# scrubbbbs/cbird

Hardware: AMD Instinct MI355X
Metric: Hamming comparisons/sec + images hashed/sec, 1M-image index, 1/2/4/8 MI355X (higher is better)
Workload: dtype u64 hashes as 64 x FP4 signs, f32 accumulate (find, exact) / u8+f32 (hash)

## Files before the change

### cbird_amd/csrc/hamm64_mfma.hip

```cpp
#include <algorithm>
#include <mutex>
#include <vector>

#include "cbh_internal.h"
#include "fp4_sign.h"

namespace cbh {
namespace {

typedef _Float16 h2 __attribute__((ext_vector_type(2)));

constexpr int kThreads = 256;
constexpr int kWaves = 4;
constexpr int kHT = 8;
constexpr int kG = 2;
constexpr float kC0 = 8388608.0f + 16448.0f + 2097152.0f;
constexpr int kScale15 = 0x8e8e8e8e;
constexpr uint32_t kQueue = 2048;
constexpr uint32_t kFlagMaskPre = (1u << 5) | (1u << 11) | (1u << 17) | (1u << 23);
constexpr int kScaleHalf = 0x7e7e7e7e;
constexpr int kScale5 = (int)0x84848484;
constexpr int kScale11 = (int)0x8a8a8a8a;
constexpr int kScale17 = (int)0x90909090;

__global__ __launch_bounds__(256) void k_expand_needles(const uint64_t* __restrict__ q, uint32_t nq,
                                                        uint32_t nq_pad, uint4* __restrict__ qx) {
  const uint32_t i = blockIdx.x * 256u + threadIdx.x;
  if (i >= 3u * nq_pad) return;
  const uint32_t* w = reinterpret_cast<const uint32_t*>(q);
  if (i < 2u * nq_pad) {
    qx[i] = fp4_expand32((i >> 1) < nq ? w[i] : 0u);
  } else {
    const uint32_t j = i - 2u * nq_pad;
    qx[i] = fp4_expand32(j < nq ? w[2u * j] ^ w[2u * j + 1u] : 0u);
  }
}

__device__ __forceinline__ h2 as_h2(float f) { return __builtin_bit_cast(h2, f); }
__device__ __forceinline__ uint32_t as_u32(float f) { return __builtin_bit_cast(uint32_t, f); }
__device__ __forceinline__ h2 pkmax3(h2 a, h2 b, h2 c) {
  return __builtin_elementwise_maximum(__builtin_elementwise_maximum(a, b), c);
}
__device__ __forceinline__ void wave_order() {
  asm volatile("" ::: "memory");
  __builtin_amdgcn_wave_barrier();
  asm volatile("" ::: "memory");
}

struct HitParams {
  uint32_t lo_key, hi_key, lo_zero, hi_zero, thresh, n, nq, keep0;
  const uint64_t* q;
  const uint32_t* ids;
  cbh_record* rec;
  unsigned long long cap;
  unsigned long long* total;
  const uint2* hay;
  const uint2* qmask;
};

constexpr uint32_t kOutCap = 128;
__device__ __forceinline__ void out_flush(uint32_t* s_out, uint32_t& nout, const HitParams& hp) {
  if (nout == 0) return;
  wave_order();
  const uint32_t lane = threadIdx.x & 63u;
  unsigned long long base = 0;
  if (lane == 0) base = atomicAdd(hp.total, (unsigned long long)nout);
  const uint32_t blo = (uint32_t)__builtin_amdgcn_readfirstlane((int)(uint32_t)base);
  const uint32_t bhi = (uint32_t)__builtin_amdgcn_readfirstlane((int)(uint32_t)(base >> 32));
  base = ((unsigned long long)bhi << 32) | blo;
  for (uint32_t k = lane; k < nout; k += 64u) {
    const uint2 r = *reinterpret_cast<const uint2*>(&s_out[2u * k]);
    if (base + k < hp.cap) hp.rec[base + k] = ((cbh_record)r.y << 32) | r.x;
  }
  wave_order();
  nout = 0;
}
__device__ __forceinline__ void out_push(uint32_t* s_out, uint32_t& nout, bool has, uint32_t qidx, uint32_t dist,
                                         uint32_t id, const HitParams& hp) {
  const uint64_t m = __builtin_amdgcn_ballot_w64(has);
  if (m == 0) return;
  const uint32_t c = (uint32_t)__popcll(m);
  if (nout + c > kOutCap) out_flush(s_out, nout, hp);
  if (has) {
    const uint32_t pos = nout + __builtin_amdgcn_mbcnt_hi((uint32_t)(m >> 32), __builtin_amdgcn_mbcnt_lo((uint32_t)m, 0u));
    *reinterpret_cast<uint2*>(&s_out[2u * pos]) = make_uint2(id, (qidx << 7) | dist);
  }
  nout += c;
}

__device__ __forceinline__ bool mask_ok(const HitParams& hp, uint32_t row, uint32_t qi, uint64_t nv) {
  if (!hp.qmask) return true;
  const uint2 hv = hp.hay[row], mk = hp.qmask[qi];
  return (((hv.x ^ (uint32_t)nv) & mk.x) | ((hv.y ^ (uint32_t)(nv >> 32)) & mk.y)) == 0;
}

__device__ __forceinline__ void handle_tile2(const v16f& c, uint32_t row0, uint32_t p, const HitParams& hp,
                                             uint32_t* s_queue, uint32_t* s_out, uint32_t& nout) {
  const uint32_t lane = threadIdx.x & 63u;
  {
    h2 m0 = {0, 0}, m1 = {0, 0};
#pragma unroll
    for (int g = 0; g < 16; g += 4) {
      m0 = pkmax3(m0, as_h2(c[g]), as_h2(c[g + 1]));
      m1 = pkmax3(m1, as_h2(c[g + 2]), as_h2(c[g + 3]));
    }
    const uint32_t tb = __builtin_bit_cast(uint32_t, __builtin_elementwise_maximum(m0, m1));
    if (__builtin_amdgcn_ballot_w64((tb << 16) >= hp.lo_key || tb >= hp.hi_key) == 0) return;
  }
  uint32_t cnt = 0;
#pragma unroll
  for (int g = 0; g < 16; ++g) {
    const uint32_t bits = as_u32(c[g]);
    const bool fh = bits >= hp.hi_key;
    const bool fl = (bits << 16) >= hp.lo_key;
    if (__builtin_amdgcn_ballot_w64(fh || fl) == 0) continue;
    const uint64_t mh = __builtin_amdgcn_ballot_w64(fh);
    if (fh)
      s_queue[cnt + __builtin_amdgcn_mbcnt_hi((uint32_t)(mh >> 32), __builtin_amdgcn_mbcnt_lo((uint32_t)mh, 0u))] =
          ((hp.hi_zero - (bits >> 16)) << 11) | (1u << 10) | ((uint32_t)g << 6) | lane;
    cnt += (uint32_t)__popcll(mh);
    const uint64_t ml = __builtin_amdgcn_ballot_w64(fl);
    if (fl)
      s_queue[cnt + __builtin_amdgcn_mbcnt_hi((uint32_t)(ml >> 32), __builtin_amdgcn_mbcnt_lo((uint32_t)ml, 0u))] =
          (((hp.lo_zero - (bits & 0xffffu)) >> 1) << 11) | ((uint32_t)g << 6) | lane;
    cnt += (uint32_t)__popcll(ml);
  }
  wave_order();
  for (uint32_t k0 = 0; k0 < cnt; k0 += 64u) {
    const uint32_t k = k0 + lane;
    const uint32_t e = s_queue[min(k, cnt - 1u)];
    const uint32_t src = e & 63u, g = (e >> 6) & 15u, field = (e >> 10) & 1u;
    const uint32_t rit = (g & 3u) + 8u * (g >> 2) + 4u * (src >> 5);
    const uint32_t row = row0 + rit;
    const uint32_t qi = p * 64u + field * 32u + (src & 31u);
    const uint32_t d = e >> 11;
    bool has = false;
    uint32_t id = 0;
    if (k < cnt && row < hp.n && qi < hp.nq) {
      const uint64_t nv = hp.q[qi];
      if (nv != 0 && d < hp.thresh && mask_ok(hp, row, qi, nv)) {
        id = hp.ids[row];
        has = id != 0 || hp.keep0;
      }
    }
    out_push(s_out, nout, has, qi, d, id, hp);
  }
  wave_order();
}

constexpr uint32_t kParkLanes = 16;
constexpr uint32_t kPark = kQueue - kParkLanes * 32u;
constexpr uint32_t kOutOff = kPark - 2u * kOutCap;
static_assert(kOutOff / 2u >= 63u + (kHT / kG) * 32u, "pending list: one-lane groups of a step");
static_assert(kOutOff / 2u >= 63u + kParkLanes * 32u, "pending list: a chunk of hit lanes");

template <int A, int B, int G>
__device__ __forceinline__ uint32_t or_regs(const v16f (&c)[G]) {
  static_assert(B - A >= 3, "range");
  uint32_t o = as_u32(c[A >> 4][A & 15]) | as_u32(c[(A + 1) >> 4][(A + 1) & 15]) | as_u32(c[(A + 2) >> 4][(A + 2) & 15]);
#pragma unroll
  for (int r = A + 3; r < B; r += 2)
    o |= as_u32(c[r >> 4][r & 15]) | (r + 1 < B ? as_u32(c[(r + 1) >> 4][(r + 1) & 15]) : 0u);
  return o;
}

template <bool PRE>
__global__ __launch_bounds__(kThreads, PRE ? 4 : 1) void k_hamm64_mfma(
    const uint2* __restrict__ hay, const uint32_t* __restrict__ ids, uint32_t n,
    const uint64_t* __restrict__ q, const uint4* __restrict__ qx, uint32_t nq, uint32_t n_pairs,
    uint32_t pairs_per_chunk, uint32_t thresh, cbh_record* __restrict__ rec,
    unsigned long long cap, unsigned long long* __restrict__ total, uint32_t keep0,
    const uint2* __restrict__ qmask, const uint4* __restrict__ qf) {
  constexpr int HT = kHT, G = kG;
  __shared__ uint32_t s_queue_[kWaves][kQueue];
  __shared__ uint2 s_hay_[PRE ? kWaves : 1][PRE ? HT * 32 : 1];
  __shared__ uint32_t s_out2_[PRE ? 1 : kWaves][PRE ? 1 : 2 * kOutCap];
  const uint32_t lane = threadIdx.x & 63u;
  const uint32_t wave = (uint32_t)__builtin_amdgcn_readfirstlane((int)(threadIdx.x >> 6));
  const uint32_t r = lane & 31u, half = lane >> 5;
  const uint32_t tile0 = (blockIdx.x * kWaves + wave) * HT;
  if (tile0 * 32u >= n) return;
  uint32_t* s_queue = s_queue_[wave];
  uint2* s_hay = s_hay_[PRE ? wave : 0];
  uint32_t* s_out = PRE ? s_queue + kOutOff : s_out2_[PRE ? 0 : wave];
  uint32_t nout = 0;

  v8i a[HT];
#pragma unroll
  for (int t = 0; t < HT; ++t) {
    const uint32_t row = (tile0 + t) * 32u + r;
    const uint2 hv = row < n ? hay[row] : make_uint2(0u, 0u);
    a[t] = fp4_operand(fp4_expand32(PRE ? hv.x ^ hv.y : (half ? hv.y : hv.x)));
    if (PRE && half == 0) s_hay[t * 32 + r] = hv;
  }
  wave_order();
  v16f c0;
#pragma unroll
  for (int g = 0; g < 16; ++g)
    c0[g] = PRE ? 8388608.0f + (float)((16u + (thresh - 1u)) * 266305u) : kC0;
  asm volatile("" : "+v"(c0));
  int scale_b = PRE ? (half ? kScale5 : kScaleHalf) : kScaleOne;
  int scale_b2 = PRE ? (half ? kScale17 : kScale11) : kScale15;
  asm volatile("" : "+v"(scale_b));
  asm volatile("" : "+v"(scale_b2));

  const uint32_t p0 = blockIdx.y * pairs_per_chunk;
  const uint32_t p1 = min(n_pairs, p0 + pairs_per_chunk);
  const uint4* __restrict__ qp = qx + ((size_t)p0 * 64u + r) * 2u + half;
  const uint32_t lo_zero = 0x4080u;
  const uint32_t hi_zero = 0x4B40u;
  const uint32_t lo_thr = lo_zero - 2u * (thresh - 1u);
  const uint32_t hi_thr = hi_zero - (thresh - 1u);
  const uint32_t lo_key = lo_thr << 16, hi_key = hi_thr << 16;
  const HitParams hp = {lo_key, hi_key, lo_zero, hi_zero, thresh, n, nq, keep0, q, ids, rec, cap, total, hay, qmask};

  uint32_t npend = 0;
  auto drain = [&](bool all) {
    wave_order();
    const uint32_t keep = all ? 0u : (npend & 63u);
    for (uint32_t k0 = keep; k0 < npend; k0 += 64u) {
      const uint32_t k = min(k0 + lane, npend - 1u);
      const uint32_t bits = s_queue[2u * k], w1 = s_queue[2u * k + 1u];
      const uint32_t g = w1 & 15u, tile = (w1 >> 4) & 7u, L = (w1 >> 7) & 63u, pp = p0 + 2u * (w1 >> 13);
      const uint32_t rit = (g & 3u) + 8u * (g >> 2) + 4u * (L >> 5);
      const uint32_t row = (tile0 + tile) * 32u + rit;
      uint32_t fields = ((bits >> 23) & 1u) ? 0xfu
                                            : (((bits >> 5) & 1u) | (((bits >> 11) & 1u) << 1) | (((bits >> 17) & 1u) << 2));
      if (row >= hp.n || k0 + lane >= npend) fields = 0;
      const uint2 hv = s_hay[tile * 32u + rit];
      while (__builtin_amdgcn_ballot_w64(fields != 0) != 0) {
        const uint32_t qi = pp * 64u + (uint32_t)__builtin_ctz(fields | 16u) * 32u + (L & 31u);
        bool has = false;
        uint32_t d = 0, id = 0;
        if (fields != 0 && qi < hp.nq) {
          const uint64_t nv = hp.q[qi];
          d = __popc(hv.x ^ (uint32_t)nv) + __popc(hv.y ^ (uint32_t)(nv >> 32));
          if (nv != 0 && d < hp.thresh && mask_ok(hp, row, qi, nv)) {
            id = hp.ids[row];
            has = id != 0 || hp.keep0;
          }
        }
        out_push(s_out, nout, has, qi, d, id, hp);
        fields &= fields - 1u;
      }
    }
    wave_order();
    npend = keep;
  };

  auto step = [&](const uint32_t p, const uint4& nA, const uint4& nB) __attribute__((always_inline)) {
    const v8i bA = fp4_operand(nA);
    const v8i bB = fp4_operand(nB);
#pragma unroll
    for (int t0 = 0; t0 < HT; t0 += G) {
      v16f c[G];
#pragma unroll
      for (int t = 0; t < G; ++t)
        c[t] = __builtin_amdgcn_mfma_scale_f32_32x32x64_f8f6f4(a[t0 + t], bA, c0, 4, 4, 0, kScaleOne,
                                                               0, scale_b);
#pragma unroll
      for (int t = 0; t < G; ++t)
        c[t] = __builtin_amdgcn_mfma_scale_f32_32x32x64_f8f6f4(a[t0 + t], bB, c[t], 4, 4, 0,
                                                               kScaleOne, 0, scale_b2);
      if constexpr (PRE) {
        constexpr int R = G * 16;
        constexpr int RA = R / 2 + 1;
        const uint32_t half0 = or_regs<0, RA, G>(c), half1 = or_regs<RA, R, G>(c);
        const uint32_t flags = (half0 | half1) & kFlagMaskPre;
        const uint64_t hm = __builtin_amdgcn_ballot_w64(flags != 0);
        if (hm != 0) {
          static_assert(R == 32, "the parking slots below are 32 registers");
          auto park4 = [&](uint32_t at, int t, int k) {
            *reinterpret_cast<float4*>(&s_queue[at + (uint32_t)(t * 16 + 4 * k)]) =
                make_float4(c[t][4 * k], c[t][4 * k + 1], c[t][4 * k + 2], c[t][4 * k + 3]);
          };
          auto park = [&](uint32_t at) {
#pragma unroll
            for (int t = 0; t < G; ++t)
#pragma unroll
              for (int k = 0; k < 4; ++k) park4(at, t, k);
          };
          const uint32_t w1c = ((uint32_t)t0 << 4) | (((p - p0) >> 1) << 13);
          auto list = [&](uint32_t at, uint32_t L, uint32_t ok) {
            uint32_t ln = lane;
            asm volatile("" : "+v"(ln));
            const uint32_t v = s_queue[at + ln];
            const bool pred = (v & kFlagMaskPre) != 0 && ((ok >> (ln & 31u)) & 1u) != 0u;
            const uint32_t bm = (uint32_t)(__builtin_amdgcn_ballot_w64(pred) & 0xffffffffull);
            if (pred && ln < (uint32_t)R) {
              *reinterpret_cast<uint2*>(&s_queue[2u * (npend + __builtin_amdgcn_mbcnt_lo(bm, 0u))]) =
                  make_uint2(v, ln | (w1c | (L << 7)));
            }
            npend += (uint32_t)__popc(bm);
          };
          if ((hm & (hm - 1)) == 0) {
            const uint64_t b0 = __builtin_amdgcn_ballot_w64((half0 & kFlagMaskPre) != 0);
            const uint64_t b1 = __builtin_amdgcn_ballot_w64((half1 & kFlagMaskPre) != 0);
            if (flags != 0) {
              if (b0) {
#pragma unroll
                for (int k = 0; k < 4; ++k) park4(kPark, 0, k);
              }
              park4(kPark, 1, 0);
              if (b1) {
#pragma unroll
                for (int k = 1; k < 4; ++k) park4(kPark, 1, k);
              }
            }
            const uint32_t ok = (b0 ? 0x000fffffu : 0u) | (b1 ? 0xffff0000u : 0u);
            wave_order();
            list(kPark, (uint32_t)__builtin_ctzll(hm), ok);
            wave_order();
          } else {
            uint64_t rest = hm;
            for (;;) {
              if (rest ? npend + kParkLanes * 32u > kOutOff / 2u : npend >= 64u) drain(false);
              if (!rest) break;
              uint64_t cm = rest;
              if ((uint32_t)__popcll(rest) > kParkLanes) {
                uint64_t rem = rest;
                for (uint32_t i = 0; i < kParkLanes; ++i) rem &= rem - 1;
                cm = rest ^ rem;
              }
              rest ^= cm;
              if ((cm >> lane) & 1ull)
                park(kPark + 32u * __builtin_amdgcn_mbcnt_hi((uint32_t)(cm >> 32), __builtin_amdgcn_mbcnt_lo((uint32_t)cm, 0u)));
              wave_order();
              uint32_t at = kPark;
              for (uint64_t m = cm; m; m &= m - 1, at += 32u) list(at, (uint32_t)__builtin_ctzll(m), 0xffffffffu);
              wave_order();
            }
          }
        }
      } else {
        h2 m0 = {0, 0}, m1 = {0, 0};
#pragma unroll
        for (int t = 0; t < G; ++t)
#pragma unroll
          for (int g = 0; g < 16; g += 4) {
            m0 = pkmax3(m0, as_h2(c[t][g]), as_h2(c[t][g + 1]));
            m1 = pkmax3(m1, as_h2(c[t][g + 2]), as_h2(c[t][g + 3]));
          }
        const uint32_t mb = __builtin_bit_cast(uint32_t, __builtin_elementwise_maximum(m0, m1));
        const bool hit = (mb << 16) >= lo_key || mb >= hi_key;
        if (__builtin_amdgcn_ballot_w64(hit) != 0) {
#pragma unroll
          for (int t = 0; t < G; ++t) handle_tile2(c[t], (tile0 + t0 + t) * 32u, p, hp, s_queue, s_out, nout);
        }
      }
    }
    if constexpr (PRE)
      if (npend >= 64u) drain(false);
  };

  if constexpr (PRE) {
    typedef unsigned v4u_t __attribute__((ext_vector_type(4)));
    const __amdgpu_buffer_rsrc_t rsrc = __builtin_amdgcn_make_buffer_rsrc(
        const_cast<uint4*>(qf + (size_t)p0 * 64u), 0, (int)0xffffffffu, 0x27000);
    const uint32_t voff = lane * 16u;
    auto ldt = [&](uint32_t rel, uint32_t partner) -> uint4 {
      const uint32_t pr = min(rel + partner, n_pairs - 1u - p0);
      const v4u_t v = __builtin_amdgcn_raw_buffer_load_b128(rsrc, (int)voff, (int)(pr * 1024u), 0);
      return make_uint4(v.x, v.y, v.z, v.w);
    };
    const uint32_t np = p1 - p0;
    uint4 a0 = ldt(0, 0), a1 = ldt(0, 1);
#pragma unroll 1
    for (uint32_t rel = 0; rel < np; rel += 4) {
      const uint4 b0 = ldt(min(rel + 2, np - 1), 0), b1 = ldt(min(rel + 2, np - 1), 1);
      step(p0 + rel, a0, a1);
      if (rel + 2 < np) {
        a0 = ldt(min(rel + 4, np - 1), 0);
        a1 = ldt(min(rel + 4, np - 1), 1);
        step(p0 + rel + 2, b0, b1);
      }
    }
    if (npend) drain(true);
  } else {
    uint4 x0 = qp[0], x1 = qp[64];
    uint32_t p = p0;
    for (; p + 1 < p1; p += 2) {
      const uint4 y0 = qp[128], y1 = qp[192];
      step(p, x0, x1);
      qp += 256;
      if (p + 2 < p1) {
        x0 = qp[0];
        x1 = qp[64];
      }
      step(p + 1, y0, y1);
    }
    if (p < p1) step(p, x0, x1);
  }
  out_flush(s_out, nout, hp);
}


constexpr uint32_t kFlagMask3 = (1u << 7) | (1u << 14) | (1u << 21);
constexpr int kScale7 = (int)0x86868686;
constexpr int kScale14 = (int)0x8d8d8d8d;

__device__ __forceinline__ void handle_tile3(const v16f& c, uint32_t row0, uint32_t p3, const HitParams& hp,
                                             uint32_t* s_queue, uint32_t* s_out, uint32_t& nout) {
  const uint32_t lane = threadIdx.x & 63u;
  uint32_t any = 0;
#pragma unroll
  for (int g = 0; g < 16; ++g) any |= as_u32(c[g]);
  if (__builtin_amdgcn_ballot_w64((any & kFlagMask3) != 0) == 0) return;
  const uint32_t b = hp.thresh - 1u;
#pragma unroll 1
  for (uint32_t f = 0; f < 3; ++f) {
    uint32_t cnt = 0;
#pragma unroll
    for (int g = 0; g < 16; ++g) {
      const uint32_t bits = as_u32(c[g]);
      const bool fl = (bits >> (7u + 7u * f)) & 1u;
      const uint64_t m = __builtin_amdgcn_ballot_w64(fl);
      if (m == 0) continue;
      if (fl)
        s_queue[cnt + __builtin_amdgcn_mbcnt_hi((uint32_t)(m >> 32), __builtin_amdgcn_mbcnt_lo((uint32_t)m, 0u))] =
            ((64u + b - ((bits >> (1u + 7u * f)) & 0x7fu)) << 12) | (f << 10) | ((uint32_t)g << 6) | lane;
      cnt += (uint32_t)__popcll(m);
    }
    wave_order();
    for (uint32_t k0 = 0; k0 < cnt; k0 += 64u) {
      const uint32_t k = k0 + lane;
      const uint32_t e = s_queue[min(k, cnt - 1u)];
      const uint32_t src = e & 63u, g = (e >> 6) & 15u, field = (e >> 10) & 3u, d = e >> 12;
      const uint32_t row = row0 + (g & 3u) + 8u * (g >> 2) + 4u * (src >> 5);
      const uint32_t qi = p3 * 96u + field * 32u + (src & 31u);
      const uint64_t nv = (k < cnt && row < hp.n && qi < hp.nq) ? hp.q[qi] : 0;
      bool has = false;
      uint32_t id = 0;
      if (nv != 0 && mask_ok(hp, row, qi, nv)) {
        id = hp.ids[row];
        has = id != 0 || hp.keep0;
      }
      out_push(s_out, nout, has, qi, d, id, hp);
    }
    wave_order();
  }
}

__global__ __launch_bounds__(kThreads, 2) void k_hamm64_mfma3(
    const uint2* __restrict__ hay, const uint32_t* __restrict__ ids, uint32_t n,
    const uint64_t* __restrict__ q, const uint4* __restrict__ qx, uint32_t nq, uint32_t n_triples,
    uint32_t triples_per_chunk, uint32_t thresh, cbh_record* __restrict__ rec,
    unsigned long long cap, unsigned long long* __restrict__ total, uint32_t keep0,
    const uint2* __restrict__ qmask) {
  constexpr int HT = kHT, G = kG;
  __shared__ uint32_t s_queue_[kWaves][16 * 64];
  __shared__ uint32_t s_out_[kWaves][2 * kOutCap];
  const uint32_t lane = threadIdx.x & 63u, wave = threadIdx.x >> 6;
  const uint32_t r = lane & 31u, half = lane >> 5;
  const uint32_t tile0 = (blockIdx.x * kWaves + wave) * HT;
  if (tile0 * 32u >= n) return;
  uint32_t* s_queue = s_queue_[wave];
  uint32_t* s_out = s_out_[wave];
  uint32_t nout = 0;

  v8i a[HT];
#pragma unroll
  for (int t = 0; t < HT; ++t) {
    const uint32_t row = (tile0 + t) * 32u + r;
    const uint2 hv = row < n ? hay[row] : make_uint2(0u, 0u);
    a[t] = fp4_operand(fp4_expand32(half ? hv.y : hv.x));
  }
  const uint32_t b = thresh - 1u;
  v16f c0;
#pragma unroll
  for (int g = 0; g < 16; ++g) c0[g] = 8388608.0f + (float)((64u + 2u * b) * 16513u);
  asm volatile("" : "+v"(c0));
  const HitParams hp = {0, 0, 0, 0, thresh, n, nq, keep0, q, ids, rec, cap, total, hay, qmask};

  const uint32_t p0 = blockIdx.y * triples_per_chunk;
  const uint32_t p1 = min(n_triples, p0 + triples_per_chunk);

  auto step = [&](const uint32_t p, const uint4& n0, const uint4& n1, const uint4& n2) __attribute__((always_inline)) {
    const v8i b0 = fp4_operand(n0), b1 = fp4_operand(n1), b2 = fp4_operand(n2);
#pragma unroll
    for (int t0 = 0; t0 < HT; t0 += G) {
      v16f c[G];
#pragma unroll
      for (int t = 0; t < G; ++t)
        c[t] = __builtin_amdgcn_mfma_scale_f32_32x32x64_f8f6f4(a[t0 + t], b0, c0, 4, 4, 0, kScaleOne, 0,
                                                               kScaleOne);
#pragma unroll
      for (int t = 0; t < G; ++t)
        c[t] = __builtin_amdgcn_mfma_scale_f32_32x32x64_f8f6f4(a[t0 + t], b1, c[t], 4, 4, 0, kScaleOne, 0,
                                                               kScale7);
#pragma unroll
      for (int t = 0; t < G; ++t)
        c[t] = __builtin_amdgcn_mfma_scale_f32_32x32x64_f8f6f4(a[t0 + t], b2, c[t], 4, 4, 0, kScaleOne, 0,
                                                               kScale14);
      if (__builtin_amdgcn_ballot_w64((or_regs<0, G * 16, G>(c) & kFlagMask3) != 0) != 0) {
#pragma unroll
        for (int t = 0; t < G; ++t) handle_tile3(c[t], (tile0 + t0 + t) * 32u, p, hp, s_queue, s_out, nout);
      }
    }
  };

  typedef unsigned v4u_t __attribute__((ext_vector_type(4)));
  const __amdgpu_buffer_rsrc_t rsrc = __builtin_amdgcn_make_buffer_rsrc(
      const_cast<uint4*>(qx + (size_t)p0 * 192u), 0, (int)0xffffffffu, 0x27000);
  const uint32_t voff = (2u * r + half) * 16u;
  auto ldt = [&](uint32_t rel, uint32_t tile) -> uint4 {
    const v4u_t v = __builtin_amdgcn_raw_buffer_load_b128(rsrc, (int)voff, (int)(rel * 3072u + tile * 1024u), 0);
    return make_uint4(v.x, v.y, v.z, v.w);
  };
  const uint32_t np = p1 - p0;
  uint4 x0 = ldt(0, 0), x1 = ldt(0, 1), x2 = ldt(0, 2);
#pragma unroll 1
  for (uint32_t rel = 0; rel < np; rel += 2) {
    const uint32_t ry = min(rel + 1, np - 1);
    const uint4 y0 = ldt(ry, 0), y1 = ldt(ry, 1), y2 = ldt(ry, 2);
    step(p0 + rel, x0, x1, x2);
    if (rel + 1 < np) {
      const uint32_t rx = min(rel + 2, np - 1);
      x0 = ldt(rx, 0);
      x1 = ldt(rx, 1);
      x2 = ldt(rx, 2);
      step(p0 + rel + 1, y0, y1, y2);
    }
  }
  out_flush(s_out, nout, hp);
}

constexpr uint32_t kProbeS = 2048;
constexpr int kProbeT = kProbeMaxThresh;

__device__ __forceinline__ uint32_t probe_mix(uint32_t x) {
  x = ((x >> 16) ^ x) * 0x45d9f3bu;
  x = ((x >> 16) ^ x) * 0x45d9f3bu;
  return (x >> 16) ^ x;
}
__global__ __launch_bounds__(256) void k_fold_probe(const uint2* __restrict__ hay, uint32_t n, const uint2* __restrict__ q,
                                                    uint32_t nq, uint32_t sh, uint32_t sq, uint32_t* __restrict__ counts) {
  __shared__ uint2 s_h[64];
  __shared__ uint32_t s_cnt[2 * kProbeT];
  const uint32_t t = threadIdx.x;
  if (t < 64) {
    const uint32_t i = blockIdx.y * 64u + t;
    s_h[t] = i < sh ? hay[sh == n ? i : probe_mix(i) % n] : make_uint2(0u, 0u);
  }
  if (t < 2 * kProbeT) s_cnt[t] = 0;
  __syncthreads();
  const uint32_t j = blockIdx.x * 256u + t;
  const uint32_t nslots = min(64u, sh - blockIdx.y * 64u);
  uint32_t cnt[kProbeT] = {}, cnt64[kProbeT] = {};
  if (j < sq) {
    const uint2 nv = q[sq == nq ? j : probe_mix(j ^ 0x9e3779b9u) % nq];
    const uint32_t f = nv.x ^ nv.y;
    for (uint32_t k = 0; k < nslots; ++k) {
      const uint2 hv = s_h[k];
      const uint32_t d = (uint32_t)__popc(f ^ hv.x ^ hv.y);
#pragma unroll
      for (int th = 0; th < kProbeT; ++th) cnt[th] += d < (uint32_t)(th + 1) ? 1u : 0u;
      if (d < (uint32_t)kProbeT) {
        const uint32_t d64 = (uint32_t)__popc(nv.x ^ hv.x) + (uint32_t)__popc(nv.y ^ hv.y);
#pragma unroll
        for (int th = 0; th < kProbeT; ++th) cnt64[th] += d64 < (uint32_t)(th + 1) ? 1u : 0u;
      }
    }
  }
#pragma unroll
  for (int th = 0; th < 2 * kProbeT; ++th) {
    uint32_t v = th < kProbeT ? cnt[th % kProbeT] : cnt64[th % kProbeT];
#pragma unroll
    for (int o = 32; o > 0; o >>= 1) v += __shfl_down(v, o);
    if ((t & 63u) == 0 && v) atomicAdd(&s_cnt[th], v);
  }
  __syncthreads();
  if (t < 2 * kProbeT && s_cnt[t]) atomicAdd(&counts[t], s_cnt[t]);
}

std::mutex g_probe_mu;
std::vector<uint32_t*> g_probe_free;
uint32_t* probe_slot_get() {
  {
    std::lock_guard<std::mutex> lk(g_probe_mu);
    if (!g_probe_free.empty()) {
      uint32_t* p = g_probe_free.back();
      g_probe_free.pop_back();
      return p;
    }
  }
  uint32_t* p = nullptr;
  if (hipHostMalloc(&p, 2 * kProbeT * sizeof(uint32_t)) != hipSuccess) {
    (void)hipGetLastError();
    return nullptr;
  }
  return p;
}
void probe_slot_put(uint32_t* p) {
  std::lock_guard<std::mutex> lk(g_probe_mu);
  g_probe_free.push_back(p);
}

}

bool probe_fold_rates(const uint64_t* d_hashes, size_t n, const uint64_t* d_q, size_t nq, int thresh, hipStream_t stream,
                      double* r_cand, double* r_true) {
  uint32_t* d_cnt = nullptr;
  if (cbh::malloc_async((void**)&d_cnt, 2 * kProbeT * sizeof(uint32_t), stream) != hipSuccess) {
    (void)hipGetLastError();
    return false;
  }
  uint32_t* h_cnt = probe_slot_get();
  bool ok = h_cnt != nullptr;
  const uint32_t sh = (uint32_t)std::min<size_t>(n, kProbeS), sq = (uint32_t)std::min<size_t>(nq, kProbeS);
  if (ok) {
    ok = hipMemsetAsync(d_cnt, 0, 2 * kProbeT * sizeof(uint32_t), stream) == hipSuccess;
    if (ok) {
      hipLaunchKernelGGL(k_fold_probe, dim3((sq + 255u) / 256u, (sh + 63u) / 64u), dim3(256), 0, stream,
                         reinterpret_cast<const uint2*>(d_hashes), (uint32_t)n, reinterpret_cast<const uint2*>(d_q),
                         (uint32_t)nq, sh, sq, d_cnt);
      ok = hipGetLastError() == hipSuccess &&
           hipMemcpyAsync(h_cnt, d_cnt, 2 * kProbeT * sizeof(uint32_t), hipMemcpyDeviceToHost, stream) == hipSuccess &&
           hipStreamSynchronize(stream) == hipSuccess;
    }
  }
  (void)cbh::free_async(d_cnt, stream);
  if (ok) {
    const double pairs = (double)sh * (double)sq;
    *r_cand = (double)h_cnt[thresh - 1] / pairs;
    *r_true = (double)h_cnt[kProbeT + thresh - 1] / pairs;
  } else {
    (void)hipGetLastError();
  }
  if (h_cnt) probe_slot_put(h_cnt);
  return ok;
}

static uint32_t padded_needles(size_t nq) { return (uint32_t)((nq + 191) / 192) * 192u; }

int expand_needles_for_scan(const uint64_t* d_q, size_t nq, hipStream_t stream, uint4** qx_out) {
  *qx_out = nullptr;
  if (nq == 0 || nq > CBH_MAX_QUERIES_PER_CALL) return CBH_OK;
  const uint32_t nq_pad = padded_needles(nq);
  uint4* qx = nullptr;
  CBH_HIP(malloc_async((void**)&qx, (size_t)nq_pad * 48u, stream));
  hipLaunchKernelGGL(k_expand_needles, dim3((3u * nq_pad + 255u) / 256u), dim3(256), 0, stream, d_q,
                     (uint32_t)nq, nq_pad, qx);
  hipError_t e = hipGetLastError();
  if (e != hipSuccess) {
    (void)free_async(qx, stream);
    CBH_HIP(e);
  }
  *qx_out = qx;
  return CBH_OK;
}

int launch_hamm64_scan_mfma(const uint64_t* d_hashes, const uint32_t* d_ids, size_t n, const uint64_t* d_q, size_t nq,
                            int thresh, cbh_record* d_rec, size_t cap, unsigned long long* d_total, hipStream_t stream,
                            bool pre, const ScanOpts& o) {
  const uint32_t n_pairs = (uint32_t)((nq + 63) / 64);
  const uint32_t n_triples = (uint32_t)((nq + 95) / 96);
  const uint32_t nq_pad = padded_needles(nq);
  const uint4* qx = o.qx;
  uint4* qx_own = nullptr;
  if (!qx) {
    int rc = expand_needles_for_scan(d_q, nq, stream, &qx_own);
    if (rc) return rc;
    qx = qx_own;
  }
  const uint4* qf = qx + 2u * (size_t)nq_pad;
  const uint32_t rows_per_wg = 32u * kHT * kWaves;
  const uint32_t sib = std::max(1u, o.siblings);
  const uint32_t wgs = (uint32_t)((n + rows_per_wg - 1) / rows_per_wg);
  if (!pre && thresh <= 64) {
    uint32_t tpc = 172u;
    while (tpc > 11 && (uint64_t)wgs * sib * ((n_triples + tpc - 1) / tpc) < 8192) tpc = (tpc + 1) / 2;
    uint32_t ch3 = (n_triples + tpc - 1) / tpc;
    if (ch3 > 65535) {
      tpc = (n_triples + 65534) / 65535;
      ch3 = (n_triples + tpc - 1) / tpc;
    }
    hipLaunchKernelGGL(k_hamm64_mfma3, dim3(wgs, ch3), dim3(kThreads), 0, stream,
                       reinterpret_cast<const uint2*>(d_hashes), d_ids, (uint32_t)n, d_q, qx, (uint32_t)nq, n_triples, tpc,
                       (uint32_t)thresh, d_rec, (unsigned long long)cap, d_total, (uint32_t)o.keep_id0,
                       reinterpret_cast<const uint2*>(o.d_qmask));
  } else {
    uint32_t ppc = pre ? 512u : 256u;
    while (ppc > 16 && (uint64_t)wgs * sib * ((n_pairs + ppc - 1) / ppc) < 8192) ppc >>= 1;
    uint32_t chunks = (n_pairs + ppc - 1) / ppc;
    if (chunks > 65535) {
      ppc = ((n_pairs + 65534) / 65535 + 1u) & ~1u;
      chunks = (n_pairs + ppc - 1) / ppc;
    }
#define CBH_MFMA(PRE)                                                                                                 \
  hipLaunchKernelGGL((k_hamm64_mfma<PRE>), dim3(wgs, chunks), dim3(kThreads), 0, stream,                              \
                     reinterpret_cast<const uint2*>(d_hashes), d_ids, (uint32_t)n, d_q, qx, (uint32_t)nq, n_pairs, ppc, \
                     (uint32_t)thresh, d_rec, (unsigned long long)cap, d_total, (uint32_t)o.keep_id0,                 \
                     reinterpret_cast<const uint2*>(o.d_qmask), qf)
    if (pre) CBH_MFMA(true); else CBH_MFMA(false);
#undef CBH_MFMA
  }
  hipError_t e = hipGetLastError();
  if (qx_own) (void)cbh::free_async(qx_own, stream);
  CBH_HIP(e);
  return CBH_OK;
}

}
```

### cbird_amd/csrc/hamm64_scan.hip

```cpp
#include <atomic>

#include "cbh_internal.h"

namespace cbh {
namespace {

constexpr int kThreads = 256;
constexpr int kH = 8;
constexpr int kQB = 8;

__device__ __forceinline__ uint32_t min3u(uint32_t a, uint32_t b, uint32_t c) {
  return min(min(a, b), c);
}

__device__ __forceinline__ void emit(cbh_record* __restrict__ rec, unsigned long long cap,
                                     unsigned long long* __restrict__ total, uint32_t qidx,
                                     uint32_t dist, uint32_t id) {
  unsigned long long slot = atomicAdd(total, 1ull);
  if (slot < cap) rec[slot] = ((cbh_record)qidx << 39) | ((cbh_record)dist << 32) | id;
}

template <int H>
__device__ __forceinline__ void exact_block(const uint2 (&h)[H], uint32_t base_idx, uint32_t n,
                                            const uint32_t* __restrict__ ids,
                                            const uint64_t* __restrict__ q, uint32_t qa,
                                            uint32_t qb, uint32_t thresh,
                                            cbh_record* __restrict__ rec, unsigned long long cap,
                                            unsigned long long* __restrict__ total,
                                            uint32_t keep0, const uint2* __restrict__ qmask) {
#pragma unroll 1
  for (uint32_t qi = qa; qi < qb; ++qi) {
    const uint64_t qq = q[qi];
    if (qq == 0) continue;
    const uint32_t ql = (uint32_t)qq, qh = (uint32_t)(qq >> 32);
    const uint2 mk = qmask ? qmask[qi] : make_uint2(0u, 0u);
#pragma unroll
    for (int j = 0; j < H; ++j) {
      const uint32_t d = __popc(h[j].x ^ ql) + __popc(h[j].y ^ qh);
      if (d < thresh && (((h[j].x ^ ql) & mk.x) | ((h[j].y ^ qh) & mk.y)) == 0) {
        const uint32_t idx = base_idx + (uint32_t)j * kThreads;
        if (idx < n) {
          const uint32_t id = ids[idx];
          if (id != 0 || keep0) emit(rec, cap, total, qi, d, id);
        }
      }
    }
  }
}

template <int H, int QB>
__device__ __forceinline__ void refine_block(const uint2 (&h)[H], const uint32_t (&acc)[H],
                                             const uint2 (&cur)[QB], uint32_t base_idx, uint32_t n,
                                             const uint32_t* __restrict__ ids, uint32_t qb,
                                             uint32_t thresh, cbh_record* __restrict__ rec,
                                             unsigned long long cap,
                                             unsigned long long* __restrict__ total,
                                             uint32_t keep0, const uint2* __restrict__ qmask) {
#pragma unroll
  for (int j = 0; j < H; ++j) {
    if (acc[j] < thresh) {
      const uint32_t idx = base_idx + (uint32_t)j * kThreads;
      uint32_t d[QB];
#pragma unroll
      for (int i = 0; i < QB; ++i) d[i] = __popc(h[j].x ^ cur[i].x) + __popc(h[j].y ^ cur[i].y);
      uint32_t m = d[0];
#pragma unroll
      for (int i = 1; i + 1 < QB; i += 2) m = min3u(m, d[i], d[i + 1]);
      if (QB % 2 == 0) m = min(m, d[QB - 1]);
      if (m < thresh && idx < n) {
        const uint32_t id = ids[idx];
        if (id != 0 || keep0) {
#pragma unroll
          for (int i = 0; i < QB; ++i)
            if (d[i] < thresh && (cur[i].x | cur[i].y) != 0) {
              const uint2 mk = qmask ? qmask[qb + (uint32_t)i] : make_uint2(0u, 0u);
              if ((((h[j].x ^ cur[i].x) & mk.x) | ((h[j].y ^ cur[i].y) & mk.y)) == 0)
                emit(rec, cap, total, qb + (uint32_t)i, d[i], id);
            }
        }
      }
    }
  }
}

enum { MODE_PRE = 0, MODE_FULL = 1, MODE_EQ = 2 };

template <int H, int QB, int MODE>
__global__ __launch_bounds__(kThreads) void k_hamm64_scan(
    const uint2* __restrict__ hay, const uint32_t* __restrict__ ids, uint32_t n,
    const uint64_t* __restrict__ q, uint32_t nq, uint32_t q_chunk, uint32_t thresh,
    cbh_record* __restrict__ rec, unsigned long long cap, unsigned long long* __restrict__ total,
    uint32_t keep0, const uint2* __restrict__ qmask) {
  const uint32_t base_idx = blockIdx.x * (uint32_t)(kThreads * H) + threadIdx.x;
  uint2 h[H];
#pragma unroll
  for (int j = 0; j < H; ++j) {
    const uint32_t idx = base_idx + (uint32_t)j * kThreads;
    h[j] = idx < n ? hay[idx] : make_uint2(0u, 0u);
  }
  const uint32_t q0 = blockIdx.y * q_chunk;
  const uint32_t q1 = min(nq, q0 + q_chunk);
  uint32_t qb = q0;
  const uint2* __restrict__ qp = reinterpret_cast<const uint2*>(q) + (size_t)q0;

  uint2 cur[QB];
  if (qb + QB <= q1) {
#pragma unroll
    for (int i = 0; i < QB; ++i) cur[i] = qp[i];
  }
  for (; qb + QB <= q1; qb += QB) {
    uint2 nxt[QB];
    qp += QB;
    if (qb + 2 * QB <= q1) {
#pragma unroll
      for (int i = 0; i < QB; ++i) nxt[i] = qp[i];
    } else {
#pragma unroll
      for (int i = 0; i < QB; ++i) nxt[i] = make_uint2(0u, 0u);
    }
    if (MODE == MODE_EQ) {
      unsigned long long any = 0;
#pragma unroll
      for (int i = 0; i < QB; ++i) {
        const unsigned long long qq = ((unsigned long long)cur[i].y << 32) | cur[i].x;
#pragma unroll
        for (int j = 0; j < H; ++j) {
          const unsigned long long hh = ((unsigned long long)h[j].y << 32) | h[j].x;
          any |= __ballot(hh == qq);
        }
      }
      if (any) exact_block<H>(h, base_idx, n, ids, q, qb, qb + QB, thresh, rec, cap, total, keep0, qmask);
    } else {
      uint32_t acc[H];
#pragma unroll
      for (int j = 0; j < H; ++j) acc[j] = 0xffu;
      uint32_t ql[QB], qh[QB];
#pragma unroll
      for (int i = 0; i < QB; ++i) {
        asm volatile("v_mov_b32 %0, %1" : "=v"(ql[i]) : "s"(cur[i].x));
        if (MODE == MODE_FULL) asm volatile("v_mov_b32 %0, %1" : "=v"(qh[i]) : "s"(cur[i].y));
      }
      uint32_t x[QB][H];
      __builtin_amdgcn_sched_barrier(0);
#pragma unroll
      for (int i = 0; i < QB; ++i)
#pragma unroll
        for (int j = 0; j < H; ++j) x[i][j] = h[j].x ^ ql[i];
      __builtin_amdgcn_sched_barrier(0);
      if (MODE == MODE_FULL) {
#pragma unroll
        for (int i = 0; i < QB; ++i)
#pragma unroll
          for (int j = 0; j < H; ++j) x[i][j] = (uint32_t)__popc(x[i][j]);
        uint32_t y[QB][H];
        __builtin_amdgcn_sched_barrier(0);
#pragma unroll
        for (int i = 0; i < QB; ++i)
#pragma unroll
          for (int j = 0; j < H; ++j) y[i][j] = h[j].y ^ qh[i];
        __builtin_amdgcn_sched_barrier(0);
#pragma unroll
        for (int i = 0; i < QB; i += 2)
#pragma unroll
          for (int j = 0; j < H; ++j)
            acc[j] = min3u(acc[j], x[i][j] + (uint32_t)__popc(y[i][j]),
                           x[i + 1][j] + (uint32_t)__popc(y[i + 1][j]));
      } else {
#pragma unroll
        for (int i = 0; i < QB; i += 2)
#pragma unroll
          for (int j = 0; j < H; ++j)
            acc[j] = min3u(acc[j], (uint32_t)__popc(x[i][j]), (uint32_t)__popc(x[i + 1][j]));
      }
      __builtin_amdgcn_sched_barrier(0);
      uint32_t m = acc[0];
#pragma unroll
      for (int j = 1; j + 1 < H; j += 2) m = min3u(m, acc[j], acc[j + 1]);
      if (H % 2 == 0) m = min(m, acc[H - 1]);
      if (m < thresh) refine_block<H, QB>(h, acc, cur, base_idx, n, ids, qb, thresh, rec, cap, total, keep0, qmask);
    }
#pragma unroll
    for (int i = 0; i < QB; ++i) cur[i] = nxt[i];
  }
  if (qb < q1) exact_block<H>(h, base_idx, n, ids, q, qb, q1, thresh, rec, cap, total, keep0, qmask);
}

constexpr unsigned kLoneSlots = 8;
__global__ __launch_bounds__(256) void k_find_one(const uint2* __restrict__ hay, const uint32_t* __restrict__ ids,
                                                  uint32_t n, uint32_t qlo, uint32_t qhi, uint32_t thresh,
                                                  unsigned* __restrict__ d_state, LoneBlock* __restrict__ host,
                                                  unsigned long long seq) {
  const uint32_t base = blockIdx.x * (256u * kLoneSlots) + threadIdx.x;
  bool wrote = false;
#pragma unroll
  for (unsigned k = 0; k < kLoneSlots; ++k) {
    const uint32_t i = base + k * 256u;
    if (i >= n) break;
    const uint2 hv = hay[i];
    const uint32_t d = (uint32_t)__popc(hv.x ^ qlo) + (uint32_t)__popc(hv.y ^ qhi);
    if (d < thresh) {
      const uint32_t id = ids[i];
      if (id != 0) {
        const unsigned slot = atomicAdd(&d_state[0], 1u);
        if (slot < LoneBlock::kRecs) {
          host->recs[slot] = ((cbh_record)d << 32) | id;
          wrote = true;
        }
      }
    }
  }
  if (wrote) __threadfence_system();
  __syncthreads();
  if (threadIdx.x == 0) {
    __threadfence();
    if (atomicAdd(&d_state[1], 1u) == gridDim.x - 1u) {
      __threadfence();
      host->count = atomicExch(&d_state[0], 0u);
      d_state[1] = 0u;
      __threadfence_system();
      __hip_atomic_store(const_cast<unsigned long long*>(&host->done), seq, __ATOMIC_RELEASE, __HIP_MEMORY_SCOPE_SYSTEM);
    }
  }
}

}

int launch_find_one(const uint64_t* d_hashes, const uint32_t* d_ids, size_t n, uint64_t q, int thresh, unsigned* d_state,
                    LoneBlock* h_block, unsigned long long seq, hipStream_t stream) {
  if (n == 0 || n > 0xfffffff0ull || !d_state || !h_block || thresh <= 0) return CBH_E_INVAL;
  const unsigned per_wg = 256u * kLoneSlots;
  hipLaunchKernelGGL(k_find_one, dim3((unsigned)((n + per_wg - 1) / per_wg)), dim3(256), 0, stream,
                     reinterpret_cast<const uint2*>(d_hashes), d_ids, (uint32_t)n, (uint32_t)q, (uint32_t)(q >> 32),
                     (uint32_t)thresh, d_state, h_block, seq);
  CBH_HIP(hipGetLastError());
  return CBH_OK;
}

int wait_find_one(const LoneBlock* h_block, unsigned long long seq, hipStream_t stream) {
  const unsigned long long* flag = const_cast<const unsigned long long*>(&h_block->done);
  for (unsigned spins = 0;; ++spins) {
    if (__atomic_load_n(flag, __ATOMIC_ACQUIRE) == seq) return CBH_OK;
    if ((spins & 0xfffu) == 0xfffu) {
      const hipError_t q = hipStreamQuery(stream);
      if (q == hipSuccess) {
        return __atomic_load_n(flag, __ATOMIC_ACQUIRE) == seq ? CBH_OK : CBH_E_HIP;
      }
      if (q != hipErrorNotReady) {
        set_last_error("k_find_one", q);
        return CBH_E_HIP;
      }
    }
#if defined(__x86_64__)
    __builtin_ia32_pause();
#endif
  }
}

namespace {

constexpr int kPreMax = 7;
constexpr size_t kMfmaMinNq = 256;
constexpr size_t kMfmaMinN = 4096;
constexpr int kPreStatic = 6;
constexpr double kTrueWeight = 4.0;
constexpr uint64_t kProbeMinPairs = 1ull << 31;

int g_scan_mfma = 1;
int g_pre_max_thresh = -1;
int g_pre_rate_max_e9 = 125000;
std::atomic<uint64_t> g_pre_mask{0};
std::atomic<uint64_t> g_n_probe{0};
std::atomic<long long> g_last_rate_e9{-1};
std::atomic<long long> g_last_true_e9{-1};

enum class Join { None, IfCheaper, Forced };
enum class Kernel { PopcEq, PopcPre, PopcFull, Mfma };
struct Route {
  Join join;
  Kernel kernel;
  double scan_ms;
};

Route route(size_t n, size_t nq, int thresh, bool masked) {
  Route r;
  r.scan_ms = (double)n * (double)nq * (thresh <= 6 ? 8.8e-12 : 16.3e-12);
  const bool joinable = thresh <= kJoinMaxThresh && !masked && n < 0xfffffff0ull;
  r.join = !joinable ? Join::None : g_scan_mfma == 4 ? Join::Forced
           : g_scan_mfma == 3 && r.scan_ms >= 1.0 ? Join::IfCheaper : Join::None;
  const bool mfma = thresh <= 65 && (g_scan_mfma == 2 || g_scan_mfma == 4 ||
                                     (g_scan_mfma != 0 && nq >= kMfmaMinNq && n >= kMfmaMinN));
  r.kernel = mfma ? Kernel::Mfma : thresh == 1 ? Kernel::PopcEq : thresh <= kPreMax ? Kernel::PopcPre : Kernel::PopcFull;
  return r;
}

int launch_popc(Kernel kernel, const uint64_t* d_hashes, const uint32_t* d_ids, size_t n, const uint64_t* d_q, size_t nq,
                int thresh, cbh_record* d_rec, size_t cap, unsigned long long* d_total, hipStream_t stream,
                const ScanOpts& o) {
  const uint32_t tile = kThreads * kH;
  const uint32_t tiles = (uint32_t)((n + tile - 1) / tile);
  uint32_t q_chunk = 16384;
  while (q_chunk > 1024 && (uint64_t)tiles * ((nq + q_chunk - 1) / q_chunk) < 8192) q_chunk >>= 1;
  uint32_t chunks = (uint32_t)((nq + q_chunk - 1) / q_chunk);
  if (chunks > 65535) {
    q_chunk = (uint32_t)((nq + 65534) / 65535);
    q_chunk = (q_chunk + kQB - 1) / kQB * kQB;
    chunks = (uint32_t)((nq + q_chunk - 1) / q_chunk);
  }
  dim3 grid(tiles, chunks), block(kThreads);
  const uint2* hay = reinterpret_cast<const uint2*>(d_hashes);
#define CBH_SCAN(MODE)                                                                                                  \
  hipLaunchKernelGGL((k_hamm64_scan<kH, kQB, MODE>), grid, block, 0, stream, hay, d_ids, (uint32_t)n, d_q, (uint32_t)nq, \
                     q_chunk, (uint32_t)thresh, d_rec, (unsigned long long)cap, d_total, (uint32_t)o.keep_id0,            \
                     reinterpret_cast<const uint2*>(o.d_qmask))
  if (kernel == Kernel::PopcEq) CBH_SCAN(MODE_EQ);
  else if (kernel == Kernel::PopcPre) CBH_SCAN(MODE_PRE);
  else CBH_SCAN(MODE_FULL);
#undef CBH_SCAN
  CBH_HIP(hipGetLastError());
  return CBH_OK;
}

}

bool scan_takes_mfma(size_t n, size_t nq, int thresh) {
  return thresh >= 1 && route(n, nq, thresh, false).kernel == Kernel::Mfma;
}

bool scan_pick_pre(const uint64_t* d_hashes, size_t n, size_t n_total, const uint64_t* d_q, size_t nq, int thresh,
                   hipStream_t stream) {
  if (thresh > 32) return false;
  if (g_pre_max_thresh >= 0) return thresh <= g_pre_max_thresh;
  if (thresh > kProbeMaxThresh) return false;
  if ((uint64_t)n_total * (uint64_t)nq < kProbeMinPairs) return thresh <= kPreStatic;
  double r_cand = 0, r_true = 0;
  if (!probe_fold_rates(d_hashes, n, d_q, nq, thresh, stream, &r_cand, &r_true)) return thresh <= kPreStatic;
  g_last_rate_e9 = (long long)(r_cand * 1e9);
  g_last_true_e9 = (long long)(r_true * 1e9);
  g_n_probe++;
  return (r_cand - kTrueWeight * r_true) * 1e9 <= (double)g_pre_rate_max_e9;
}

int launch_hamm64_scan(const uint64_t* d_hashes, const uint32_t* d_ids, size_t n, const uint64_t* d_q, size_t nq,
                       int thresh, cbh_record* d_rec, size_t cap, unsigned long long* d_total, hipStream_t stream,
                       const ScanOpts& o) {
  if (n == 0 || nq == 0 || thresh <= 0) return CBH_OK;
  if (n > 0xfffffff0ull || nq > CBH_MAX_QUERIES_PER_CALL) return CBH_E_INVAL;
  const Route r = route(n, nq, thresh, o.d_qmask != nullptr);
  if (r.join != Join::None) {
    const bool force = r.join == Join::Forced;
    const int rc = launch_hamm64_join(d_hashes, d_ids, n, d_q, nq, thresh, d_rec, cap, d_total, stream, o.keep_id0, force,
                                      r.scan_ms);
    if (rc == CBH_OK || force || (rc != CBH_E_UNSUPPORTED && rc != CBH_E_NOMEM)) return rc;
    if (rc == CBH_E_NOMEM) cbh_clear_error();
  }
  if (r.kernel != Kernel::Mfma) return launch_popc(r.kernel, d_hashes, d_ids, n, d_q, nq, thresh, d_rec, cap, d_total, stream, o);
  const bool pre = o.pre >= 0 ? o.pre != 0 : scan_pick_pre(d_hashes, n, n, d_q, nq, thresh, stream);
  if (thresh < 64) {
    if (pre) g_pre_mask |= 1ull << thresh; else g_pre_mask &= ~(1ull << thresh);
  }
  return launch_hamm64_scan_mfma(d_hashes, d_ids, n, d_q, nq, thresh, d_rec, cap, d_total, stream, pre, o);
}

int set_scan_mfma(int mode) {
  if (mode < 0 || mode > 4) return CBH_E_INVAL;
  g_scan_mfma = mode;
  return CBH_OK;
}
int get_scan_mfma() { return g_scan_mfma; }
void set_scan_pre_max(int t) {
  if (t >= -1 && t <= 32) g_pre_max_thresh = t;
}
void set_scan_pre_rate(int e9) {
  if (e9 >= 0) g_pre_rate_max_e9 = e9;
}
long long get_scan_pre_mask() { return (long long)g_pre_mask.load(); }
long long get_scan_probes() { return (long long)g_n_probe.load(); }
long long get_scan_probe_rate_e9() { return g_last_rate_e9.load(); }
long long get_scan_probe_true_e9() { return g_last_true_e9.load(); }

}
```

Measured before the change: 78410 billion.

## Replace register parking with compact per-lane hit descriptors in prefilter MFMA kernel

```diff
diff --git a/cbird_amd/csrc/hamm64_mfma.hip b/cbird_amd/csrc/hamm64_mfma.hip
--- a/cbird_amd/csrc/hamm64_mfma.hip
+++ b/cbird_amd/csrc/hamm64_mfma.hip
@@ -148,11 +148,12 @@
   wave_order();
 }
 
-constexpr uint32_t kParkLanes = 16;
-constexpr uint32_t kPark = kQueue - kParkLanes * 32u;
-constexpr uint32_t kOutOff = kPark - 2u * kOutCap;
-static_assert(kOutOff / 2u >= 63u + (kHT / kG) * 32u, "pending list: one-lane groups of a step");
-static_assert(kOutOff / 2u >= 63u + kParkLanes * 32u, "pending list: a chunk of hit lanes");
+constexpr uint32_t kPendCap = 320;
+constexpr uint32_t kOutOff = 2u * kPendCap;
+constexpr uint32_t kPreQueue = kOutOff + 2u * kOutCap;
+static_assert(kPendCap >= 63u + (kHT / kG) * 64u, "pending list: every lane of every group of a step");
+static_assert(kPreQueue <= kQueue, "the prefilter kernel's LDS must not grow");
+static_assert(kG == 2, "a descriptor names the two reduction chains of a group of 32 registers");
 
 template <int A, int B, int G>
 __device__ __forceinline__ uint32_t or_regs(const v16f (&c)[G]) {
@@ -172,8 +173,8 @@
     unsigned long long cap, unsigned long long* __restrict__ total, uint32_t keep0,
     const uint2* __restrict__ qmask, const uint4* __restrict__ qf) {
   constexpr int HT = kHT, G = kG;
-  __shared__ uint32_t s_queue_[kWaves][kQueue];
-  __shared__ uint2 s_hay_[PRE ? kWaves : 1][PRE ? HT * 32 : 1];
+  __shared__ __attribute__((aligned(16))) uint32_t s_queue_[kWaves][PRE ? kPreQueue : kQueue];
+  __shared__ __attribute__((aligned(16))) uint2 s_hay_[PRE ? kWaves : 1][PRE ? HT * 32 : 1];
   __shared__ uint32_t s_out2_[PRE ? 1 : kWaves][PRE ? 1 : 2 * kOutCap];
   const uint32_t lane = threadIdx.x & 63u;
   const uint32_t wave = (uint32_t)__builtin_amdgcn_readfirstlane((int)(threadIdx.x >> 6));
@@ -220,28 +221,62 @@
     const uint32_t keep = all ? 0u : (npend & 63u);
     for (uint32_t k0 = keep; k0 < npend; k0 += 64u) {
       const uint32_t k = min(k0 + lane, npend - 1u);
-      const uint32_t bits = s_queue[2u * k], w1 = s_queue[2u * k + 1u];
-      const uint32_t g = w1 & 15u, tile = (w1 >> 4) & 7u, L = (w1 >> 7) & 63u, pp = p0 + 2u * (w1 >> 13);
-      const uint32_t rit = (g & 3u) + 8u * (g >> 2) + 4u * (L >> 5);
-      const uint32_t row = (tile0 + tile) * 32u + rit;
-      uint32_t fields = ((bits >> 23) & 1u) ? 0xfu
-                                            : (((bits >> 5) & 1u) | (((bits >> 11) & 1u) << 1) | (((bits >> 17) & 1u) << 2));
-      if (row >= hp.n || k0 + lane >= npend) fields = 0;
-      const uint2 hv = s_hay[tile * 32u + rit];
-      while (__builtin_amdgcn_ballot_w64(fields != 0) != 0) {
-        const uint32_t qi = pp * 64u + (uint32_t)__builtin_ctz(fields | 16u) * 32u + (L & 31u);
-        bool has = false;
-        uint32_t d = 0, id = 0;
-        if (fields != 0 && qi < hp.nq) {
-          const uint64_t nv = hp.q[qi];
-          d = __popc(hv.x ^ (uint32_t)nv) + __popc(hv.y ^ (uint32_t)(nv >> 32));
-          if (nv != 0 && d < hp.thresh && mask_ok(hp, row, qi, nv)) {
+      const uint2 e = *reinterpret_cast<const uint2*>(&s_queue[2u * k]);
+      const uint32_t L = e.y & 63u, pp = p0 + 2u * (e.y >> 8);
+      const uint32_t base = ((e.y >> 6) & 3u) * 64u + 4u * (L >> 5);
+      const uint32_t col = pp * 64u + (L & 31u);
+      uint32_t cm = 0;
+#pragma unroll
+      for (uint32_t c = 0; c < 2; ++c) {
+        const uint32_t w = e.x >> c;
+        cm |= (((w >> 23) & 1u) ? 0xfu : (((w >> 5) & 1u) | (((w >> 11) & 1u) << 1) | (((w >> 17) & 1u) << 2))) << (4u * c);
+      }
+      if (k0 + lane >= npend) cm = 0;
+      uint32_t nlo[4], nhi[4];
+#pragma unroll
+      for (uint32_t f = 0; f < 4; ++f) {
+        const uint64_t nv = (((cm | (cm >> 4)) >> f) & 1u) != 0 && col + 32u * f < hp.nq ? hp.q[col + 32u * f] : 0;
+        nlo[f] = (uint32_t)nv;
+        nhi[f] = (uint32_t)(nv >> 32);
+      }
+#pragma unroll
+      for (uint32_t f = 0; f < 4; ++f)
+        if ((nlo[f] | nhi[f]) == 0) cm &= ~(0x11u << f);
+      while (__builtin_amdgcn_ballot_w64(cm != 0) != 0) {
+        const uint32_t b = (uint32_t)__builtin_ctz(cm | 0x100u), f = b & 3u, ch = (b >> 2) & 1u;
+        const uint32_t qlo = f == 0 ? nlo[0] : f == 1 ? nlo[1] : f == 2 ? nlo[2] : nlo[3];
+        const uint32_t qhi = f == 0 ? nhi[0] : f == 1 ? nhi[1] : f == 2 ? nhi[2] : nhi[3];
+        const uint32_t rows = cm == 0 ? 0u : ch ? 0xfffe0000u : 0x0001ffffu;
+        const uint2* hq = s_hay + base + 32u * ch;
+        uint32_t hit = 0;
+#pragma unroll 1
+        for (uint32_t i = 0; i < 5u; ++i) {
+          const uint32_t qd = 4u * ch + i;
+          const uint4* h4 = reinterpret_cast<const uint4*>(hq + 8u * min(i, 4u - ch));
+          const uint4 x = h4[0], y = h4[1];
+          const uint32_t d0 = __popc(x.x ^ qlo) + __popc(x.y ^ qhi), d1 = __popc(x.z ^ qlo) + __popc(x.w ^ qhi);
+          const uint32_t d2 = __popc(y.x ^ qlo) + __popc(y.y ^ qhi), d3 = __popc(y.z ^ qlo) + __popc(y.w ^ qhi);
+          const uint32_t m4 = (d0 < hp.thresh ? 1u : 0u) | (d1 < hp.thresh ? 2u : 0u) | (d2 < hp.thresh ? 4u : 0u) |
+                              (d3 < hp.thresh ? 8u : 0u);
+          hit |= qd < 8u ? m4 << (4u * qd) : 0u;
+        }
+        hit &= rows;
+        const uint32_t qi = col + 32u * f;
+        while (__builtin_amdgcn_ballot_w64(hit != 0) != 0) {
+          const uint32_t rr = (uint32_t)__builtin_ctz(hit | 0x80000000u);
+          const uint32_t wr = base + 8u * (rr >> 2) + (rr & 3u), row = tile0 * 32u + wr;
+          const uint2 hv = s_hay[wr];
+          const uint32_t d = __popc(hv.x ^ qlo) + __popc(hv.y ^ qhi);
+          bool has = false;
+          uint32_t id = 0;
+          if (hit != 0 && row < hp.n && mask_ok(hp, row, qi, ((uint64_t)qhi << 32) | qlo)) {
             id = hp.ids[row];
             has = id != 0 || hp.keep0;
           }
+          out_push(s_out, nout, has, qi, d, id, hp);
+          hit &= hit - 1u;
         }
-        out_push(s_out, nout, has, qi, d, id, hp);
-        fields &= fields - 1u;
+        cm &= cm - 1u;
       }
     }
     wave_order();
@@ -269,68 +304,16 @@
         const uint32_t flags = (half0 | half1) & kFlagMaskPre;
         const uint64_t hm = __builtin_amdgcn_ballot_w64(flags != 0);
         if (hm != 0) {
-          static_assert(R == 32, "the parking slots below are 32 registers");
-          auto park4 = [&](uint32_t at, int t, int k) {
-            *reinterpret_cast<float4*>(&s_queue[at + (uint32_t)(t * 16 + 4 * k)]) =
-                make_float4(c[t][4 * k], c[t][4 * k + 1], c[t][4 * k + 2], c[t][4 * k + 3]);
-          };
-          auto park = [&](uint32_t at) {
-#pragma unroll
-            for (int t = 0; t < G; ++t)
-#pragma unroll
-              for (int k = 0; k < 4; ++k) park4(at, t, k);
-          };
-          const uint32_t w1c = ((uint32_t)t0 << 4) | (((p - p0) >> 1) << 13);
-          auto list = [&](uint32_t at, uint32_t L, uint32_t ok) {
-            uint32_t ln = lane;
-            asm volatile("" : "+v"(ln));
-            const uint32_t v = s_queue[at + ln];
-            const bool pred = (v & kFlagMaskPre) != 0 && ((ok >> (ln & 31u)) & 1u) != 0u;
-            const uint32_t bm = (uint32_t)(__builtin_amdgcn_ballot_w64(pred) & 0xffffffffull);
-            if (pred && ln < (uint32_t)R) {
-              *reinterpret_cast<uint2*>(&s_queue[2u * (npend + __builtin_amdgcn_mbcnt_lo(bm, 0u))]) =
-                  make_uint2(v, ln | (w1c | (L << 7)));
-            }
-            npend += (uint32_t)__popc(bm);
-          };
-          if ((hm & (hm - 1)) == 0) {
-            const uint64_t b0 = __builtin_amdgcn_ballot_w64((half0 & kFlagMaskPre) != 0);
-            const uint64_t b1 = __builtin_amdgcn_ballot_w64((half1 & kFlagMaskPre) != 0);
-            if (flags != 0) {
-              if (b0) {
-#pragma unroll
-                for (int k = 0; k < 4; ++k) park4(kPark, 0, k);
-              }
-              park4(kPark, 1, 0);
-              if (b1) {
-#pragma unroll
-                for (int k = 1; k < 4; ++k) park4(kPark, 1, k);
-              }
-            }
-            const uint32_t ok = (b0 ? 0x000fffffu : 0u) | (b1 ? 0xffff0000u : 0u);
-            wave_order();
-            list(kPark, (uint32_t)__builtin_ctzll(hm), ok);
-            wave_order();
-          } else {
-            uint64_t rest = hm;
-            for (;;) {
-              if (rest ? npend + kParkLanes * 32u > kOutOff / 2u : npend >= 64u) drain(false);
-              if (!rest) break;
-              uint64_t cm = rest;
-              if ((uint32_t)__popcll(rest) > kParkLanes) {
-                uint64_t rem = rest;
-                for (uint32_t i = 0; i < kParkLanes; ++i) rem &= rem - 1;
-                cm = rest ^ rem;
-              }
-              rest ^= cm;
-              if ((cm >> lane) & 1ull)
-                park(kPark + 32u * __builtin_amdgcn_mbcnt_hi((uint32_t)(cm >> 32), __builtin_amdgcn_mbcnt_lo((uint32_t)cm, 0u)));
-              wave_order();
-              uint32_t at = kPark;
-              for (uint64_t m = cm; m; m &= m - 1, at += 32u) list(at, (uint32_t)__builtin_ctzll(m), 0xffffffffu);
-              wave_order();
-            }
+          static_assert(R == 32, "two chains of 17 and 15 registers");
+          uint32_t ln = lane;
+          asm volatile("" : "+v"(ln));
+          if (flags != 0) {
+            const uint32_t at = __builtin_amdgcn_mbcnt_hi((uint32_t)(hm >> 32), __builtin_amdgcn_mbcnt_lo((uint32_t)hm, npend));
+            *reinterpret_cast<uint2*>(&s_queue[2u * at]) =
+                make_uint2((half0 & kFlagMaskPre) | ((half1 & kFlagMaskPre) << 1),
+                           ln | ((uint32_t)(t0 / G) << 6) | (((p - p0) >> 1) << 8));
           }
+          npend += (uint32_t)__popcll(hm);
         }
       } else {
         h2 m0 = {0, 0}, m1 = {0, 0};
diff --git a/cbird_amd/csrc/hamm64_scan.hip b/cbird_amd/csrc/hamm64_scan.hip
--- a/cbird_amd/csrc/hamm64_scan.hip
+++ b/cbird_amd/csrc/hamm64_scan.hip
@@ -262,12 +262,12 @@
 constexpr size_t kMfmaMinNq = 256;
 constexpr size_t kMfmaMinN = 4096;
 constexpr int kPreStatic = 6;
-constexpr double kTrueWeight = 4.0;
+constexpr double kTrueWeight = 8.0;
 constexpr uint64_t kProbeMinPairs = 1ull << 31;
 
 int g_scan_mfma = 1;
 int g_pre_max_thresh = -1;
-int g_pre_rate_max_e9 = 125000;
+int g_pre_rate_max_e9 = 300000;
 std::atomic<uint64_t> g_pre_mask{0};
 std::atomic<uint64_t> g_n_probe{0};
 std::atomic<long long> g_last_rate_e9{-1};
@@ -283,7 +283,7 @@
 
 Route route(size_t n, size_t nq, int thresh, bool masked) {
   Route r;
-  r.scan_ms = (double)n * (double)nq * (thresh <= 6 ? 8.8e-12 : 16.3e-12);
+  r.scan_ms = (double)n * (double)nq * (thresh <= 5 ? 8.7e-12 : thresh == 6 ? 10.0e-12 : thresh == 7 ? 14.7e-12 : 15.8e-12);
   const bool joinable = thresh <= kJoinMaxThresh && !masked && n < 0xfffffff0ull;
   r.join = !joinable ? Join::None : g_scan_mfma == 4 ? Join::Forced
            : g_scan_mfma == 3 && r.scan_ms >= 1.0 ? Join::IfCheaper : Join::None;
```

Measured after the change: 81140 billion, median of 6. 1.03x the previous value.
